# sMedX/FaceNet

Hardware: AMD Instinct MI355X
Metric: images/sec (160x160 triplet train) (higher is better)
Workload: dtype bf16

## Files before the change

facenet_amd/csrc/common.h:

```cpp
#pragma once
#include <hip/hip_runtime.h>
#include <stdint.h>
#include <atomic>
#include <cstdlib>

namespace fn {

enum { FN_OK = 0, FN_EINVAL = -1, FN_ELAUNCH = -2, FN_EUNSUPPORTED = -3 };
void set_error(const char* fmt, ...);
int check_launch(const char* what);

#define FN_REQUIRE(cond, ...)                  \
    do {                                       \
        if (!(cond)) {                         \
            fn::set_error(__VA_ARGS__);        \
            return fn::FN_EINVAL;              \
        }                                      \
    } while (0)

typedef __attribute__((ext_vector_type(8))) __bf16 bf16x8;
typedef __attribute__((ext_vector_type(4))) __bf16 bf16x4;
typedef __attribute__((ext_vector_type(8))) _Float16 f16x8;
typedef __attribute__((ext_vector_type(4))) _Float16 f16x4;
typedef __attribute__((ext_vector_type(4))) float f32x4;
// ... 31 lines not shown
    static __device__ __forceinline__ f32x4 mfma(vec8 a, vec8 b, f32x4 c) {
        return __builtin_amdgcn_mfma_f32_16x16x32_f16(a, b, c, 0, 0, 0);
    }
};

template <typename T> __device__ __forceinline__ void unpack8(const u32x4& v, float (&f)[8]) {
#pragma unroll
    for (int i = 0; i < 4; ++i) {
        f[2 * i] = LP<T>::to_f32((unsigned short)(v[i] & 0xffffu));
        f[2 * i + 1] = LP<T>::to_f32((unsigned short)(v[i] >> 16));
    }
}
template <typename T> __device__ __forceinline__ u32x4 pack8(const float (&f)[8]) {
    u32x4 v;
#pragma unroll
    for (int i = 0; i < 4; ++i)
        v[i] = (unsigned)LP<T>::from_f32(f[2 * i]) | ((unsigned)LP<T>::from_f32(f[2 * i + 1]) << 16);
    return v;
}

__device__ __forceinline__ void fast_divmod(int m, int d, float inv, int& q, int& r) {
    q = (int)((float)m * inv);
    r = m - q * d;
    const int lo = r < 0 ? 1 : 0, hi = r >= d ? 1 : 0;
    q += hi - lo;
    r += (lo - hi) * d;
}

__device__ __forceinline__ float wave_sum(float v) {
#pragma unroll
    for (int o = 32; o > 0; o >>= 1) v += __shfl_xor(v, o);
    return v;
}
__device__ __forceinline__ float wave_max(float v) {
#pragma unroll
    for (int o = 32; o > 0; o >>= 1) v = fmaxf(v, __shfl_xor(v, o));
    return v;
}

typedef int64_t acc_t;
enum { ACC_STAT = 20, ACC_GRAD = 40 };
template <int FRAC> __device__ __forceinline__ void acc_add(acc_t* p, float v) {
    atomicAdd(reinterpret_cast<unsigned long long*>(p), (unsigned long long)__double2ll_rn((double)v * (double)(1ll << FRAC)));
}
template <int FRAC> __device__ __forceinline__ float acc_get(acc_t a) { return (float)((double)a * (1.0 / (double)(1ll << FRAC))); }

__device__ __forceinline__ void bn_affine_from_sums(float s1, float s2, int count, float eps, float beta, float& scale, float& shift,
                                                    float& mean, float& var) {
#pragma clang fp contract(off)
    const float inv = 1.f / (float)count;
    mean = s1 * inv;
    const float ex2 = s2 * inv, m2 = mean * mean;
    var = fmaxf(ex2 - m2, 0.f);
    scale = rsqrtf(var + eps);
    const float ms = mean * scale;
    shift = beta - ms;
}

__device__ __forceinline__ float bn_moving_update(float moving, float batch, float momentum) {
#pragma clang fp contract(off)
    const float a = moving * momentum, w = 1.f - momentum;
    const float b = batch * w;
    return a + b;
}

__device__ __forceinline__ void bn_batch_affine(const acc_t* __restrict__ stats, int c, int sq_off, int reps, int rep_stride, int count,
                                                float eps, float beta, float& scale, float& shift, float& mean, float& var) {
    acc_t s = 0, q = 0;
    for (int rp = 0; rp < reps; ++rp) {
        s += stats[(long)rp * rep_stride + c];
        q += stats[(long)rp * rep_stride + sq_off + c];
    }
    bn_affine_from_sums(acc_get<ACC_STAT>(s), acc_get<ACC_STAT>(q), count, eps, beta, scale, shift, mean, var);
}

enum { STORE_WT = 17 };
// ... 48 lines not shown
```

facenet_amd/csrc/elementwise.hip:

```cpp
#include "common.h"
#include "../../include/facenet_hip.h"

namespace fn {

__device__ __forceinline__ unsigned f2ord(float f) {
    unsigned u = __float_as_uint(f);
    return (u & 0x80000000u) ? ~u : (u | 0x80000000u);
}
__device__ __forceinline__ float ord2f(unsigned u) {
    return __uint_as_float((u & 0x80000000u) ? (u & 0x7fffffffu) : ~u);
}

template <typename SRC>
__global__ __launch_bounds__(256) void img_stats_kernel(const SRC* __restrict__ img, unsigned* __restrict__ work, int count) {
    const int n = blockIdx.y;
    const SRC* p = img + (long)n * count;
    float mx = -3e38f, mn = 3e38f, s = 0.f, q = 0.f;
    constexpr int PER = 16 / sizeof(SRC);
    const int head = min(count, (int)(((16 - ((uintptr_t)p & 15)) & 15) / sizeof(SRC)));
    const int nvec = (count - head) / PER;
    const SRC* pv = p + head;
    for (int i = blockIdx.x * 256 + threadIdx.x; i < nvec; i += gridDim.x * 256) {
        const u32x4 v = *reinterpret_cast<const u32x4*>(pv + (long)i * PER);
#pragma unroll
        for (int w = 0; w < 4; ++w) {
            if constexpr (sizeof(SRC) == 1) {
#pragma unroll
                for (int b = 0; b < 4; ++b) {
                    const float x = (float)((v[w] >> (8 * b)) & 0xffu);
                    mx = fmaxf(mx, x); mn = fminf(mn, x); s += x; q += x * x;
                }
            } else {
                const float x = __uint_as_float(v[w]);
                mx = fmaxf(mx, x); mn = fminf(mn, x); s += x; q += x * x;
            }
        }
    }
    if (blockIdx.x == 0) {
        for (int i = threadIdx.x; i < head; i += 256) {
            const float x = (float)p[i];
            mx = fmaxf(mx, x); mn = fminf(mn, x); s += x; q += x * x;
        }
        for (int i = head + nvec * PER + threadIdx.x; i < count; i += 256) {
            const float x = (float)p[i];
            mx = fmaxf(mx, x); mn = fminf(mn, x); s += x; q += x * x;
        }
    }
    mx = wave_max(mx); mn = -wave_max(-mn); s = wave_sum(s); q = wave_sum(q);
    if ((threadIdx.x & 63) == 0) {
        atomicMax(&work[8 * n + 0], f2ord(mx));
        atomicMax(&work[8 * n + 1], f2ord(-mn));
        acc_add<ACC_STAT>(reinterpret_cast<acc_t*>(&work[8 * n + 2]), s);
        acc_add<ACC_STAT>(reinterpret_cast<acc_t*>(&work[8 * n + 4]), q);
    }
}

template <typename T, typename SRC>
__global__ __launch_bounds__(256) void img_apply_kernel(const SRC* __restrict__ img, unsigned short* __restrict__ out,
                                                        const unsigned* __restrict__ work, int HW, int mode) {
    const int n = blockIdx.y;
    float mul, sub, den;
    if (mode == 0) {
        const float mx = ord2f(work[8 * n + 0]), mn = -ord2f(work[8 * n + 1]);
        mul = 2.f; sub = mn + mx; den = fmaxf(mx - mn, 1e-3f);
    } else {
        const float cnt = (float)HW * 3.f;
        const float mean = acc_get<ACC_STAT>(*reinterpret_cast<const acc_t*>(&work[8 * n + 2])) / cnt;
        const float var = fmaxf(acc_get<ACC_STAT>(*reinterpret_cast<const acc_t*>(&work[8 * n + 4])) / cnt - mean * mean, 0.f);
        mul = 1.f; sub = mean; den = fmaxf(sqrtf(var), rsqrtf(cnt));
    }
    const SRC* p = img + (long)n * HW * 3;
    unsigned short* o = out + (long)n * HW * 8;
    for (int px = blockIdx.x * 256 + threadIdx.x; px < HW; px += gridDim.x * 256) {
        float v[8] = {0, 0, 0, 0, 0, 0, 0, 0};
#pragma unroll
        for (int c = 0; c < 3; ++c) v[c] = (mul * (float)p[px * 3 + c] - sub) / den;
        *reinterpret_cast<u32x4*>(o + (long)px * 8) = pack8<T>(v);
    }
}

template <typename SRC>
__global__ __launch_bounds__(256) void resize_bilinear_kernel(const SRC* __restrict__ img, float* __restrict__ out, int N, int H, int W,
                                                              int OH, int OW) {
    const float sy = (float)H / (float)OH, sx = (float)W / (float)OW;
    const long total = (long)N * OH * OW;
    for (long t = (long)blockIdx.x * 256 + threadIdx.x; t < total; t += (long)gridDim.x * 256) {
        const int ox = (int)(t % OW);
        const int oy = (int)((t / OW) % OH);
        const int n = (int)(t / ((long)OW * OH));
        const float fy = ((float)oy + 0.5f) * sy - 0.5f, fx = ((float)ox + 0.5f) * sx - 0.5f;
        const float fy0 = floorf(fy), fx0 = floorf(fx);
        const int y0 = max((int)fy0, 0), y1 = min((int)ceilf(fy), H - 1);
        const int x0 = max((int)fx0, 0), x1 = min((int)ceilf(fx), W - 1);
        const float ly = fy - fy0, lx = fx - fx0;
        const SRC* p = img + (long)n * H * W * 3;
#pragma unroll
        for (int c = 0; c < 3; ++c) {
            const float v00 = (float)p[((long)y0 * W + x0) * 3 + c], v01 = (float)p[((long)y0 * W + x1) * 3 + c];
            const float v10 = (float)p[((long)y1 * W + x0) * 3 + c], v11 = (float)p[((long)y1 * W + x1) * 3 + c];
            const float top = v00 + (v01 - v00) * lx, bot = v10 + (v11 - v10) * lx;
            out[t * 3 + c] = top + (bot - top) * ly;
        }
    }
}

__global__ __launch_bounds__(256) void gather_images_kernel(const uint8_t* __restrict__ pool, const int32_t* __restrict__ idx,
                                                            uint8_t* __restrict__ out, int bytes) {
    const int i = blockIdx.y;
    const uint8_t* s = pool + (long)idx[i] * bytes;
    uint8_t* d = out + (long)i * bytes;
// ... 618 lines not shown
    }
}

template <typename T> __global__ __launch_bounds__(256) void cast_kernel(const float* __restrict__ x, unsigned short* __restrict__ y, long n) {
    for (long i = (long)blockIdx.x * 256 + threadIdx.x; i < n; i += (long)gridDim.x * 256) y[i] = LP<T>::from_f32(x[i]);
}

static inline int reduce_rows_per_block(int M, int C) {
    int chunks = 32768 / (C > 0 ? C : 1);
    if (chunks < 8) chunks = 8;
    if (chunks > 1024) chunks = 1024;
    int rpb = cdiv(M, chunks);
    if (rpb < 32) rpb = 32;
    return rpb;
}

static inline int grid_for(long work_items, int per_block = 256, int cap = 4096) {
    long g = (work_items + per_block - 1) / per_block;
    if (g < 1) g = 1;
    if (g > cap) g = cap;
    return (int)g;
}

}

using namespace fn;
#define DT_CHECK(dt) FN_REQUIRE((dt) == FN_BF16 || (dt) == FN_F16, "dtype %d unsupported", (dt))
#define LAUNCH_T(dt, KERN, grid, block, smem, st, ...)                                             \
    do {                                                                                             \
        if ((dt) == FN_BF16) hipLaunchKernelGGL(KERN<__bf16>, grid, block, smem, st, __VA_ARGS__);   \
        else hipLaunchKernelGGL(KERN<_Float16>, grid, block, smem, st, __VA_ARGS__);                 \
    } while (0)

template <typename SRC>
static int image_normalize_impl(const SRC* img, void* out, float* work, int N, int HW, int mode, int dtype, void* stream) {
    DT_CHECK(dtype);
    FN_REQUIRE(img && out && work && N > 0 && HW > 0, "image_normalize: bad arguments");
    FN_REQUIRE(mode == 0 || mode == 1, "Invalid image normalization algorithm");
    FN_REQUIRE(((uintptr_t)img % sizeof(SRC)) == 0, "image_normalize: misaligned images");
    hipStream_t st = (hipStream_t)stream;
    fill_words(work, 0u, 0u, 8 * N, st);
    hipLaunchKernelGGL(img_stats_kernel<SRC>, dim3(8, N), dim3(256), 0, st, img, (unsigned*)work, HW * 3);
    const int gx = grid_for(HW, 256, 32);
    if (dtype == FN_BF16) hipLaunchKernelGGL((img_apply_kernel<__bf16, SRC>), dim3(gx, N), dim3(256), 0, st, img, (unsigned short*)out, (const unsigned*)work, HW, mode);
    else hipLaunchKernelGGL((img_apply_kernel<_Float16, SRC>), dim3(gx, N), dim3(256), 0, st, img, (unsigned short*)out, (const unsigned*)work, HW, mode);
    return check_launch("image_normalize");
}
extern "C" int fn_image_normalize(const uint8_t* img, void* out, float* work, int N, int HW, int mode, int dtype, void* stream) {
    return image_normalize_impl<uint8_t>(img, out, work, N, HW, mode, dtype, stream);
}
extern "C" int fn_image_normalize_f32(const float* img, void* out, float* work, int N, int HW, int mode, int dtype, void* stream) {
    return image_normalize_impl<float>(img, out, work, N, HW, mode, dtype, stream);
}

extern "C" int fn_image_resize_bilinear(const void* img, int src_is_f32, float* out, int N, int H, int W, int OH, int OW, void* stream) {
    FN_REQUIRE(img && out && N > 0 && H > 0 && W > 0 && OH > 0 && OW > 0, "image_resize: bad arguments");
    const int grid = grid_for((long)N * OH * OW);
    if (src_is_f32) hipLaunchKernelGGL(resize_bilinear_kernel<float>, dim3(grid), dim3(256), 0, (hipStream_t)stream, (const float*)img, out, N, H, W, OH, OW);
    else hipLaunchKernelGGL(resize_bilinear_kernel<uint8_t>, dim3(grid), dim3(256), 0, (hipStream_t)stream, (const uint8_t*)img, out, N, H, W, OH, OW);
    return check_launch("image_resize");
}

__global__ __launch_bounds__(256) void crop_or_pad_kernel(const uint8_t* __restrict__ src, const long long* __restrict__ off,
                                                          const int* __restrict__ hw, uint8_t* __restrict__ dst, int S) {
    const int n = blockIdx.y;
    const int h = hw[2 * n], w = hw[2 * n + 1];
    const int cy = max((h - S) / 2, 0), cx = max((w - S) / 2, 0);
    const int py = max((S - h) / 2, 0), px = max((S - w) / 2, 0);
    const int ch = min(h, S), cw = min(w, S);
    const uint8_t* im = src + off[n];
    const int words = S * S * 3 / 4;
    for (int t = blockIdx.x * 256 + threadIdx.x; t < words; t += gridDim.x * 256) {
        unsigned v = 0;
#pragma unroll
        for (int b = 0; b < 4; ++b) {
// ... 213 lines not shown
```

facenet_amd/csrc/loss.hip:

```cpp
#include "pair_tiles.h"
#include "../../include/facenet_hip.h"

namespace fn {

__global__ __launch_bounds__(256) void pairwise_kernel(const float* __restrict__ xa, const float* __restrict__ xb, float* __restrict__ out,
                                                       int* __restrict__ range, int n, int m, int E, int metric) {
    const int lane = threadIdx.x & 63, wave = threadIdx.x >> 6;
    const int i = blockIdx.y;
    const int jb = (blockIdx.x * 4 + wave) * 16;
    if (jb >= m) return;
    float a[8];
#pragma unroll
    for (int t = 0; t < 8; ++t) a[t] = (lane + 64 * t < E) ? xa[(long)i * E + lane + 64 * t] : 0.f;
    float asq = 0.f;
#pragma unroll
    for (int t = 0; t < 8; ++t) asq = __fmaf_rn(a[t], a[t], asq);
    asq = wave_sum(asq);
    DotRange seen;
    for (int j = jb; j < min(m, jb + 16); ++j) {
        float d = 0.f, bsq = 0.f;
#pragma unroll
        for (int t = 0; t < 8; ++t) {
            const float b = (lane + 64 * t < E) ? xb[(long)j * E + lane + 64 * t] : 0.f;
            d = __fmaf_rn(a[t], b, d);
            bsq = __fmaf_rn(b, b, bsq);
        }
        d = wave_sum(d);
        float r;
        if (metric == 2) {
            bsq = wave_sum(bsq);
            r = fmaxf(__fmaf_rn(-2.f, d, asq + bsq), 0.f);
        } else {
            seen.add(d);
            r = pair_distance(d, metric);
        }
        if (lane == 0) out[(long)i * m + j] = r;
    }
    if (range && lane == 0 && metric != 2) seen.write(range);
}

__device__ __forceinline__ unsigned hash_mix(unsigned h, unsigned v) {
    h ^= v;
    h ^= h >> 16;
    h *= 0x7FEB352Du;
    h ^= h >> 15;
    h *= 0x846CA68Bu;
    h ^= h >> 16;
    return h;
}
__device__ __forceinline__ unsigned hash_u32(unsigned a, unsigned b, unsigned c) {
    return hash_mix(hash_mix(hash_mix(0x9E3779B9u, a), b), c);
}

__global__ __launch_bounds__(1024) void select_pairs_kernel(const int* __restrict__ labels, int n, int* __restrict__ info) {
    __shared__ int s_lab[1024];
    __shared__ int s_off[1025];
    const int tid = threadIdx.x;
    int* rec = info + 8;
    for (int i = tid; i < n; i += 1024) s_lab[i] = labels[i];
    __syncthreads();
    int cnt = 0;
    if (tid < n)
        for (int p = tid + 1; p < n; ++p) cnt += (s_lab[p] == s_lab[tid]);
    {
        __shared__ int s_wtot[16];
        const int lane = tid & 63, wv = tid >> 6;
        int v = tid < n ? cnt : 0;
#pragma unroll
        for (int d = 1; d < 64; d <<= 1) {
            const int u = __shfl_up(v, d);
            if (lane >= d) v += u;
        }
        if (lane == 63) s_wtot[wv] = v;
        __syncthreads();
        int carry = 0;
        for (int w = 0; w < wv; ++w) carry += s_wtot[w];
        if (tid < n) s_off[tid + 1] = v + carry;
        if (tid == 0) s_off[0] = 0;
    }
    __syncthreads();
    if (tid < n) {
        int q = s_off[tid];
        for (int p = tid + 1; p < n; ++p)
            if (s_lab[p] == s_lab[tid]) { rec[5 * q + 0] = tid; rec[5 * q + 1] = p; ++q; }
    }
    if (tid == 0) {
        info[0] = s_off[n];
        info[1] = 0;
    }
}

__global__ __launch_bounds__(256) void select_negatives_kernel(const float* __restrict__ dist, const int* __restrict__ labels, int n,
                                                               float alpha, unsigned seed0, int semi_hard, int* __restrict__ info) {
    const int lane = threadIdx.x & 63;
    const int q = blockIdx.x * 4 + (threadIdx.x >> 6);
    if (q >= info[0]) return;
    const unsigned seed = seed0 + (unsigned)info[3];
    int* rec = info + 8;
    const int a = rec[5 * q + 0], p = rec[5 * q + 1];
    const int la = labels[a];
    const float dap = dist[(long)p * n + a];
    int c = 0, others = 0;
    for (int j0 = 0; j0 < n; j0 += 64) {
        const int j = j0 + lane;
        const bool oth = (j < n) && (labels[j] != la);
        const float daj = oth ? dist[(long)j * n + a] : 0.f;
        const bool cand = oth && (daj - dap < alpha) && (!semi_hard || daj > dap);
        c += __popcll(__ballot(cand));
        others += __popcll(__ballot(oth));
    }
    const bool use_cand = c > 0;
    int want = use_cand ? (int)(hash_u32(seed, (unsigned)q, 0u) % (unsigned)c)
                        : (others > 0 ? (int)(hash_u32(seed, (unsigned)q, 2u) % (unsigned)others) : -1);
    int neg = -1;
    for (int j0 = 0; j0 < n && want >= 0; j0 += 64) {
        const int j = j0 + lane;
        const bool oth = (j < n) && (labels[j] != la);
        const float daj = oth ? dist[(long)j * n + a] : 0.f;
        const bool hit = use_cand ? (oth && (daj - dap < alpha) && (!semi_hard || daj > dap)) : oth;
        const unsigned long long m = __ballot(hit);
        const int cnt = __popcll(m);
        if (want < cnt) {
            const int rank = __popcll(m & ((1ull << lane) - 1ull));
            const unsigned long long sel = __ballot(hit && rank == want);
            neg = j0 + (int)__ffsll((long long)sel) - 1;
            want = -1;
        } else {
            want -= cnt;
        }
    }
    if (lane == 0) {
        rec[5 * q + 2] = neg;
        rec[5 * q + 3] = (int)hash_u32(seed, (unsigned)q, 1u);
        rec[5 * q + 4] = use_cand ? 0 : 1;
        if (use_cand) atomicAdd(&info[1], 1);
    }
}

__global__ __launch_bounds__(1024) void select_rank_kernel(int T, int* __restrict__ triplets, int* __restrict__ info) {
    const int tid = threadIdx.x;
    const int* rec = info + 8;
    const int Q = info[0];
    __shared__ unsigned long long s_key[4096];
    for (int q = tid; q < min(Q, 4096); q += 1024)
        s_key[q] = ((unsigned long long)(unsigned)rec[5 * q + 4] << 32) | (unsigned)rec[5 * q + 3];
    __syncthreads();
    for (int q = tid; q < Q; q += 1024) {
        const int cls = rec[5 * q + 4];
        const unsigned key = (unsigned)rec[5 * q + 3];
        const unsigned long long mine = ((unsigned long long)(unsigned)cls << 32) | key;
        int rank = 0;
        const int QL = min(Q, 4096);
        for (int r = 0; r < QL; ++r) {
            const unsigned long long k2 = s_key[r];
            rank += (k2 < mine || (k2 == mine && r < q)) ? 1 : 0;
        }
        for (int r = QL; r < Q; ++r) {
            const int c2 = rec[5 * r + 4];
            const unsigned k2 = (unsigned)rec[5 * r + 3];
            const bool before = (c2 < cls) || (c2 == cls && (k2 < key || (k2 == key && r < q)));
            rank += before ? 1 : 0;
        }
        if (rank < T && rec[5 * q + 2] >= 0) {
            triplets[3 * rank + 0] = rec[5 * q + 0];
            triplets[3 * rank + 1] = rec[5 * q + 1];
            triplets[3 * rank + 2] = rec[5 * q + 2];
        }
    }
    if (tid == 0) {
        info[2] = (Q < T) ? 1 : 0;
        info[3] = info[3] + 1;
    }
}

__global__ __launch_bounds__(256) void triplet_loss_kernel(const float* __restrict__ emb, float* __restrict__ demb, acc_t* __restrict__ loss,
                                                           int T, int E, float alpha) {
    const int t = blockIdx.x * 4 + (threadIdx.x >> 6), lane = threadIdx.x & 63;
    if (t >= T) return;
    const float* a = emb + (long)(3 * t) * E;
    const float* p = a + E;
    const float* ng = p + E;
    float pos = 0.f, neg = 0.f;
    for (int k = lane; k < E; k += 64) {
        const float dp = a[k] - p[k], dn = a[k] - ng[k];
        pos += dp * dp;
        neg += dn * dn;
    }
    pos = wave_sum(pos);
    neg = wave_sum(neg);
    const float l = pos - neg + alpha;
    const float on = l > 0.f ? 1.f : 0.f;
    if (lane == 0) acc_add<ACC_GRAD>(loss, fmaxf(l, 0.f) / (float)T);
    if (demb) {
        const float s = 2.f * on / (float)T;
        float* da = demb + (long)(3 * t) * E;
        for (int k = lane; k < E; k += 64) {
            da[k] = s * (ng[k] - p[k]);
            da[E + k] = s * (p[k] - a[k]);
            da[2 * E + k] = s * (a[k] - ng[k]);
        }
    }
}

template <typename T>
__global__ __launch_bounds__(256) void softmax_xent_kernel(const float* __restrict__ logits, int ld, const int* __restrict__ labels,
                                                           acc_t* __restrict__ loss, unsigned short* __restrict__ dlogits, int ld_d,
                                                           acc_t* __restrict__ dbias, int N, int C, float grad_scale) {
    __shared__ float red[4];
    const int row = blockIdx.x, tid = threadIdx.x, lane = tid & 63, wave = tid >> 6;
    const float* x = logits + (long)row * ld;
    float mx = -3e38f;
    for (int c = tid; c < C; c += 256) mx = fmaxf(mx, x[c]);
    mx = wave_max(mx);
    if (lane == 0) red[wave] = mx;
    __syncthreads();
    mx = fmaxf(fmaxf(red[0], red[1]), fmaxf(red[2], red[3]));
    __syncthreads();
    float s = 0.f;
    for (int c = tid; c < C; c += 256) s += __expf(x[c] - mx);
    s = wave_sum(s);
    if (lane == 0) red[wave] = s;
    __syncthreads();
    s = red[0] + red[1] + red[2] + red[3];
    const int lab = labels[row];
    const bool lab_ok = lab >= 0 && lab < C;
    if (tid == 0) {
        if (lab_ok) acc_add<ACC_GRAD>(loss, (logf(s) + mx - x[lab]) / (float)N);
        else reinterpret_cast<volatile unsigned*>(loss)[-1] = 1u;
    }
    if (dlogits) {
        const float inv = 1.f / s;
        unsigned short* d = dlogits + (long)row * ld_d;
        for (int c = tid; c < ld_d; c += 256) {
// ... 254 lines not shown
    const float* wr = w + (long)j * E;
    float* dr = dw + (long)j * E;
    for (int e = 4 * lane; e < E; e += 256) {
        const f32x4 wv = *reinterpret_cast<const f32x4*>(wr + e);
        f32x4 dv = *reinterpret_cast<const f32x4*>(dr + e);
#pragma unroll
        for (int t = 0; t < 4; ++t) {
            const float p = kf * wv[t];
            dv[t] = dv[t] - p;
        }
        *reinterpret_cast<f32x4*>(dr + e) = dv;
    }
}
}
using namespace fn;

extern "C" int fn_pairwise_sqdist(const float* xa, const float* xb, float* out, float* range, int n, int m, int E, int metric, void* stream) {
    FN_REQUIRE(xa && xb && out && n > 0 && m > 0 && E > 0 && E <= 512, "pairwise_sqdist: bad arguments (E must be <= 512)");
    FN_REQUIRE(metric >= 0 && metric <= 2, "Undefined similarity metric %d", metric);
    hipStream_t st = (hipStream_t)stream;
    if (range) {
        fill_words(range, 0x7f7fffffu, 0x80800000u, 2, st);
    }
    hipLaunchKernelGGL(pairwise_kernel, dim3(cdiv(m, 64), n), dim3(256), 0, st, xa, xb, out, (int*)range, n, m, E, metric);
    return check_launch("pairwise_sqdist");
}

extern "C" int fn_select_triplets(const float* dist, const int32_t* labels, int n, float alpha, int nrof_triplets, uint32_t seed,
                                  int semi_hard, int32_t* triplets, int32_t* info, void* stream) {
    FN_REQUIRE(dist && labels && triplets && info && n > 1 && n <= 1024 && nrof_triplets > 0, "select_triplets: bad arguments (n <= 1024)");
    hipStream_t st = (hipStream_t)stream;
    hipLaunchKernelGGL(select_pairs_kernel, dim3(1), dim3(1024), 0, st, labels, n, info);
    const int max_pairs = n * (n - 1) / 2;
    hipLaunchKernelGGL(select_negatives_kernel, dim3(cdiv(max_pairs, 4)), dim3(256), 0, st, dist, labels, n, alpha, seed, semi_hard, info);
    hipLaunchKernelGGL(select_rank_kernel, dim3(1), dim3(1024), 0, st, nrof_triplets, triplets, info);
    return check_launch("select_triplets");
}

extern "C" int fn_triplet_loss_fwd_bwd(const float* emb, float* demb, float* loss, int T, int E, float alpha, void* stream) {
    FN_REQUIRE(emb && loss && T > 0 && E > 0, "triplet_loss: bad arguments");
    hipStream_t st = (hipStream_t)stream;
    FN_REQUIRE(((uintptr_t)loss & 7) == 0, "triplet_loss: loss must be an 8-byte aligned fp32[4]");
    fill_words(loss, 0u, 0u, 4, st);
    hipLaunchKernelGGL(triplet_loss_kernel, dim3(cdiv(T, 4)), dim3(256), 0, st, emb, demb, reinterpret_cast<acc_t*>(loss + 2), T, E, alpha);
    hipLaunchKernelGGL(loss_finish_kernel, dim3(1), dim3(1), 0, st, loss);
    return check_launch("triplet_loss");
}

extern "C" int fn_softmax_xent_fwd_bwd(const float* logits, int ld, const int32_t* labels, float* loss, void* dlogits_lp, int ld_d, fn_acc_t* dbias_,
                                       int N, int C, float grad_scale, int dtype, void* stream) {
    acc_t* dbias = reinterpret_cast<acc_t*>(dbias_);
    FN_REQUIRE(((uintptr_t)loss & 7) == 0, "softmax_xent: loss must be an 8-byte aligned fp32[4]");
    FN_REQUIRE(dtype == FN_BF16 || dtype == FN_F16, "dtype %d unsupported", dtype);
    FN_REQUIRE(logits && labels && loss && N > 0 && C > 0 && ld >= C && (!dlogits_lp || ld_d >= C), "softmax_xent: bad arguments");
    hipStream_t st = (hipStream_t)stream;
    fill_words(loss, 0u, 0u, 4, st);
    acc_t* lacc = reinterpret_cast<acc_t*>(loss + 2);
    if (dtype == FN_BF16)
        hipLaunchKernelGGL(softmax_xent_kernel<__bf16>, dim3(N), dim3(256), 0, st, logits, ld, labels, lacc, (unsigned short*)dlogits_lp, ld_d, dbias, N, C, grad_scale);
    else
        hipLaunchKernelGGL(softmax_xent_kernel<_Float16>, dim3(N), dim3(256), 0, st, logits, ld, labels, lacc, (unsigned short*)dlogits_lp, ld_d, dbias, N, C, grad_scale);
    hipLaunchKernelGGL(loss_finish_kernel, dim3(1), dim3(1), 0, st, loss);
    return check_launch("softmax_xent");
}

extern "C" int fn_center_loss_fwd_bwd(const float* x, const int32_t* labels, const float* centers, float* demb, float* terms, float* xy,
                                      int ld_xy, int N, int E, int C, float center_factor, float norm_factor, float p, void* stream) {
    FN_REQUIRE(x && labels && terms && N > 0 && E > 0 && E % 4 == 0, "center_loss: bad arguments (E must be a multiple of 4)");
    FN_REQUIRE(((uintptr_t)x & 15) == 0 && (!demb || ((uintptr_t)demb & 15) == 0) && (!centers || ((uintptr_t)centers & 15) == 0),
               "center_loss: x, demb and centers must be 16-byte aligned");
    FN_REQUIRE(((uintptr_t)terms & 7) == 0, "center_loss: terms must be an 8-byte aligned fp32[8]");
    FN_REQUIRE(!centers || C > 0, "center_loss: centers need C > 0");
    FN_REQUIRE(!xy || ld_xy > E, "center_loss: ld_xy must be > E");
    FN_REQUIRE(center_factor >= 0.f && norm_factor >= 0.f && p > 0.f, "center_loss: factors must be >= 0 and p > 0");
    hipStream_t st = (hipStream_t)stream;
// ... 50 lines not shown
```

Measured before the change: 14110.

## Fuse image normalize, triplet selection and loss kernels to cut launches

Image normalization now runs as one kernel per image that stages the image in LDS, computes statistics and applies the affine transform, with a lookup table for 8-bit inputs. This replaces the separate fill, stats and apply launches. Negative selection and ranking are merged into one kernel that uses a last-block ticket, and pair counting uses wave ballots. The pairwise distance loop batches four wave reductions. Small triplet counts use a single-block loss kernel without the fill and finish launches. These cut launch overhead and serialization in the non-GEMM pipeline stages, but they add complexity and lower parallelism per image (one block).

```diff
diff --git a/facenet_amd/csrc/common.h b/facenet_amd/csrc/common.h
--- a/facenet_amd/csrc/common.h
+++ b/facenet_amd/csrc/common.h
@@ -87,6 +87,16 @@
     for (int o = 32; o > 0; o >>= 1) v += __shfl_xor(v, o);
     return v;
 }
+template <int N> __device__ __forceinline__ void wave_sum_n(float (&v)[N]) {
+#pragma unroll
+    for (int o = 32; o > 0; o >>= 1) {
+        float u[N];
+#pragma unroll
+        for (int k = 0; k < N; ++k) u[k] = __shfl_xor(v[k], o);
+#pragma unroll
+        for (int k = 0; k < N; ++k) v[k] += u[k];
+    }
+}
 __device__ __forceinline__ float wave_max(float v) {
 #pragma unroll
     for (int o = 32; o > 0; o >>= 1) v = fmaxf(v, __shfl_xor(v, o));
@@ -95,8 +105,9 @@
 
 typedef int64_t acc_t;
 enum { ACC_STAT = 20, ACC_GRAD = 40 };
+template <int FRAC> __device__ __forceinline__ acc_t acc_fixed(float v) { return __double2ll_rn((double)v * (double)(1ll << FRAC)); }
 template <int FRAC> __device__ __forceinline__ void acc_add(acc_t* p, float v) {
-    atomicAdd(reinterpret_cast<unsigned long long*>(p), (unsigned long long)__double2ll_rn((double)v * (double)(1ll << FRAC)));
+    atomicAdd(reinterpret_cast<unsigned long long*>(p), (unsigned long long)acc_fixed<FRAC>(v));
 }
 template <int FRAC> __device__ __forceinline__ float acc_get(acc_t a) { return (float)((double)a * (1.0 / (double)(1ll << FRAC))); }
 
diff --git a/facenet_amd/csrc/elementwise.hip b/facenet_amd/csrc/elementwise.hip
--- a/facenet_amd/csrc/elementwise.hip
+++ b/facenet_amd/csrc/elementwise.hip
@@ -10,72 +10,165 @@
 __device__ __forceinline__ float ord2f(unsigned u) {
     return __uint_as_float((u & 0x80000000u) ? (u & 0x7fffffffu) : ~u);
 }
+
+struct ImgStat {
+    float mx = -3e38f, mn = 3e38f, s = 0.f, q = 0.f;
+    __device__ __forceinline__ void add(float x) { mx = fmaxf(mx, x); mn = fminf(mn, x); s += x; q += x * x; }
+    template <typename SRC> __device__ __forceinline__ void add_vec(const u32x4& v) {
+#pragma unroll
+        for (int w = 0; w < 4; ++w) {
+            if constexpr (sizeof(SRC) == 1) {
+#pragma unroll
+                for (int b = 0; b < 4; ++b) add((float)((v[w] >> (8 * b)) & 0xffu));
+            } else {
+                add(__uint_as_float(v[w]));
+            }
+        }
+    }
+    __device__ __forceinline__ void reduce_wave() { mx = wave_max(mx); mn = -wave_max(-mn); s = wave_sum(s); q = wave_sum(q); }
+};
+
+template <typename SRC> __device__ __forceinline__ int img_head(const SRC* p, int count) {
+    return min(count, (int)(((16 - ((uintptr_t)p & 15)) & 15) / sizeof(SRC)));
+}
+
+enum { IMG_STAT_THREADS = 2048, IMG_STAT_WAVES = IMG_STAT_THREADS / 64, IMG_STAT_LDS = IMG_STAT_WAVES * 24,
+       IMG_TABLE_LDS = 256 * 2 };
 
 template <typename SRC>
 __global__ __launch_bounds__(256) void img_stats_kernel(const SRC* __restrict__ img, unsigned* __restrict__ work, int count) {
     const int n = blockIdx.y;
     const SRC* p = img + (long)n * count;
-    float mx = -3e38f, mn = 3e38f, s = 0.f, q = 0.f;
+    ImgStat st;
     constexpr int PER = 16 / sizeof(SRC);
-    const int head = min(count, (int)(((16 - ((uintptr_t)p & 15)) & 15) / sizeof(SRC)));
+    const int head = img_head(p, count);
     const int nvec = (count - head) / PER;
     const SRC* pv = p + head;
-    for (int i = blockIdx.x * 256 + threadIdx.x; i < nvec; i += gridDim.x * 256) {
-        const u32x4 v = *reinterpret_cast<const u32x4*>(pv + (long)i * PER);
-#pragma unroll
-        for (int w = 0; w < 4; ++w) {
-            if constexpr (sizeof(SRC) == 1) {
-#pragma unroll
-                for (int b = 0; b < 4; ++b) {
-                    const float x = (float)((v[w] >> (8 * b)) & 0xffu);
-                    mx = fmaxf(mx, x); mn = fminf(mn, x); s += x; q += x * x;
-                }
-            } else {
-                const float x = __uint_as_float(v[w]);
-                mx = fmaxf(mx, x); mn = fminf(mn, x); s += x; q += x * x;
-            }
-        }
-    }
+    for (int i = blockIdx.x * 256 + threadIdx.x; i < nvec; i += gridDim.x * 256)
+        st.template add_vec<SRC>(*reinterpret_cast<const u32x4*>(pv + (long)i * PER));
     if (blockIdx.x == 0) {
-        for (int i = threadIdx.x; i < head; i += 256) {
-            const float x = (float)p[i];
-            mx = fmaxf(mx, x); mn = fminf(mn, x); s += x; q += x * x;
-        }
-        for (int i = head + nvec * PER + threadIdx.x; i < count; i += 256) {
-            const float x = (float)p[i];
-            mx = fmaxf(mx, x); mn = fminf(mn, x); s += x; q += x * x;
-        }
-    }
-    mx = wave_max(mx); mn = -wave_max(-mn); s = wave_sum(s); q = wave_sum(q);
+        for (int i = threadIdx.x; i < head; i += 256) st.add((float)p[i]);
+        for (int i = head + nvec * PER + threadIdx.x; i < count; i += 256) st.add((float)p[i]);
+    }
+    st.reduce_wave();
     if ((threadIdx.x & 63) == 0) {
-        atomicMax(&work[8 * n + 0], f2ord(mx));
-        atomicMax(&work[8 * n + 1], f2ord(-mn));
-        acc_add<ACC_STAT>(reinterpret_cast<acc_t*>(&work[8 * n + 2]), s);
-        acc_add<ACC_STAT>(reinterpret_cast<acc_t*>(&work[8 * n + 4]), q);
-    }
-}
+        atomicMax(&work[8 * n + 0], f2ord(st.mx));
+        atomicMax(&work[8 * n + 1], f2ord(-st.mn));
+        acc_add<ACC_STAT>(reinterpret_cast<acc_t*>(&work[8 * n + 2]), st.s);
+        acc_add<ACC_STAT>(reinterpret_cast<acc_t*>(&work[8 * n + 4]), st.q);
+    }
+}
+
+struct ImgAffine {
+    float mul, sub, den;
+    __device__ __forceinline__ ImgAffine(unsigned omx, unsigned omn, acc_t s, acc_t q, int HW, int mode) {
+        if (mode == 0) {
+            const float mx = ord2f(omx), mn = -ord2f(omn);
+            mul = 2.f; sub = mn + mx; den = fmaxf(mx - mn, 1e-3f);
+        } else {
+            const float cnt = (float)HW * 3.f;
+            const float mean = acc_get<ACC_STAT>(s) / cnt;
+            const float var = fmaxf(acc_get<ACC_STAT>(q) / cnt - mean * mean, 0.f);
+            mul = 1.f; sub = mean; den = fmaxf(sqrtf(var), rsqrtf(cnt));
+        }
+    }
+    template <typename T, typename SRC> __device__ __forceinline__ u32x4 pixel(const SRC* p) const {
+        float v[8] = {0, 0, 0, 0, 0, 0, 0, 0};
+#pragma unroll
+        for (int c = 0; c < 3; ++c) v[c] = value((float)p[c]);
+        return pack8<T>(v);
+    }
+    __device__ __forceinline__ float value(float x) const { return (mul * x - sub) / den; }
+};
 
 template <typename T, typename SRC>
 __global__ __launch_bounds__(256) void img_apply_kernel(const SRC* __restrict__ img, unsigned short* __restrict__ out,
                                                         const unsigned* __restrict__ work, int HW, int mode) {
     const int n = blockIdx.y;
-    float mul, sub, den;
-    if (mode == 0) {
-        const float mx = ord2f(work[8 * n + 0]), mn = -ord2f(work[8 * n + 1]);
-        mul = 2.f; sub = mn + mx; den = fmaxf(mx - mn, 1e-3f);
-    } else {
-        const float cnt = (float)HW * 3.f;
-        const float mean = acc_get<ACC_STAT>(*reinterpret_cast<const acc_t*>(&work[8 * n + 2])) / cnt;
-        const float var = fmaxf(acc_get<ACC_STAT>(*reinterpret_cast<const acc_t*>(&work[8 * n + 4])) / cnt - mean * mean, 0.f);
-        mul = 1.f; sub = mean; den = fmaxf(sqrtf(var), rsqrtf(cnt));
-    }
+    const ImgAffine af(work[8 * n + 0], work[8 * n + 1], *reinterpret_cast<const acc_t*>(&work[8 * n + 2]),
+                       *reinterpret_cast<const acc_t*>(&work[8 * n + 4]), HW, mode);
     const SRC* p = img + (long)n * HW * 3;
     unsigned short* o = out + (long)n * HW * 8;
-    for (int px = blockIdx.x * 256 + threadIdx.x; px < HW; px += gridDim.x * 256) {
-        float v[8] = {0, 0, 0, 0, 0, 0, 0, 0};
-#pragma unroll
-        for (int c = 0; c < 3; ++c) v[c] = (mul * (float)p[px * 3 + c] - sub) / den;
-        *reinterpret_cast<u32x4*>(o + (long)px * 8) = pack8<T>(v);
+    for (int px = blockIdx.x * 256 + threadIdx.x; px < HW; px += gridDim.x * 256)
+        *reinterpret_cast<u32x4*>(o + (long)px * 8) = af.template pixel<T, SRC>(p + px * 3);
+}
+
+template <typename T, typename SRC>
+__global__ __launch_bounds__(1024) void img_normalize_kernel(const SRC* __restrict__ img, unsigned short* __restrict__ out,
+                                                             unsigned* __restrict__ work, int HW, int mode) {
+    extern __shared__ u32x4 s_lds[];
+    acc_t* s_s = reinterpret_cast<acc_t*>(s_lds);
+    acc_t* s_q = s_s + IMG_STAT_WAVES;
+    unsigned* s_mx = reinterpret_cast<unsigned*>(s_q + IMG_STAT_WAVES);
+    unsigned* s_mn = s_mx + IMG_STAT_WAVES;
+    unsigned short* s_tab = reinterpret_cast<unsigned short*>(s_lds + IMG_STAT_LDS / 16);
+    u32x4* s_img4 = s_lds + (IMG_STAT_LDS + IMG_TABLE_LDS) / 16;
+    const int n = blockIdx.x, tid = threadIdx.x, lane = tid & 63;
+    const int count = HW * 3;
+    const SRC* p = img + (long)n * count;
+    constexpr int PER = 16 / sizeof(SRC);
+    const int head = img_head(p, count);
+    const int nvec = (count - head) / PER;
+    SRC* s_el = reinterpret_cast<SRC*>(s_img4) + ((uintptr_t)p & 15) / sizeof(SRC);
+    u32x4* s_vec = reinterpret_cast<u32x4*>(s_el + head);
+    const u32x4* pv = reinterpret_cast<const u32x4*>(p + head);
+    for (int i0 = tid; i0 < nvec; i0 += 5 * 1024) {
+        u32x4 r[5];
+#pragma unroll
+        for (int k = 0; k < 5; ++k) r[k] = (i0 + 1024 * k < nvec) ? pv[i0 + 1024 * k] : u32x4{0u, 0u, 0u, 0u};
+#pragma unroll
+        for (int k = 0; k < 5; ++k)
+            if (i0 + 1024 * k < nvec) s_vec[i0 + 1024 * k] = r[k];
+    }
+    if (tid < 256) {
+        for (int i = tid; i < head; i += 256) s_el[i] = p[i];
+        for (int i = head + nvec * PER + tid; i < count; i += 256) s_el[i] = p[i];
+    }
+#pragma unroll
+    for (int half = 0; half < 2; ++half) {
+        const int vt = tid + 1024 * half;
+        ImgStat st;
+        for (int i = vt; i < nvec; i += IMG_STAT_THREADS) st.template add_vec<SRC>(s_vec[i]);
+        if (vt < 256) {
+            for (int i = vt; i < head; i += 256) st.add((float)s_el[i]);
+            for (int i = head + nvec * PER + vt; i < count; i += 256) st.add((float)s_el[i]);
+        }
+        st.reduce_wave();
+        if (lane == 0) {
+            const int w = vt >> 6;
+            s_mx[w] = f2ord(st.mx);
+            s_mn[w] = f2ord(-st.mn);
+            s_s[w] = acc_fixed<ACC_STAT>(st.s);
+            s_q[w] = acc_fixed<ACC_STAT>(st.q);
+        }
+    }
+    __syncthreads();
+    unsigned omx = 0u, omn = 0u;
+    acc_t ss = 0, qq = 0;
+#pragma unroll
+    for (int w = 0; w < IMG_STAT_WAVES; ++w) {
+        omx = max(omx, s_mx[w]); omn = max(omn, s_mn[w]);
+        ss += s_s[w]; qq += s_q[w];
+    }
+    if (tid == 0) {
+        unsigned* w = work + 8 * n;
+        w[0] = omx; w[1] = omn;
+        *reinterpret_cast<acc_t*>(w + 2) = ss;
+        *reinterpret_cast<acc_t*>(w + 4) = qq;
+        w[6] = 0u; w[7] = 0u;
+    }
+    const ImgAffine af(omx, omn, ss, qq, HW, mode);
+    unsigned short* o = out + (long)n * HW * 8;
+    if constexpr (sizeof(SRC) == 1) {
+        if (tid < 256) s_tab[tid] = LP<T>::from_f32(af.value((float)tid));
+        __syncthreads();
+        for (int px = tid; px < HW; px += 1024) {
+            const SRC* e = s_el + px * 3;
+            *reinterpret_cast<u32x4*>(o + (long)px * 8) = u32x4{(unsigned)s_tab[e[0]] | ((unsigned)s_tab[e[1]] << 16), (unsigned)s_tab[e[2]], 0u, 0u};
+        }
+    } else {
+        for (int px = tid; px < HW; px += 1024)
+            *reinterpret_cast<u32x4*>(o + (long)px * 8) = af.template pixel<T, SRC>(s_el + px * 3);
     }
 }
 
@@ -760,6 +853,8 @@
         else hipLaunchKernelGGL(KERN<_Float16>, grid, block, smem, st, __VA_ARGS__);                 \
     } while (0)
 
+enum { IMG_LDS_MAX_BYTES = 158 * 1024 };
+
 template <typename SRC>
 static int image_normalize_impl(const SRC* img, void* out, float* work, int N, int HW, int mode, int dtype, void* stream) {
     DT_CHECK(dtype);
@@ -767,8 +862,19 @@
     FN_REQUIRE(mode == 0 || mode == 1, "Invalid image normalization algorithm");
     FN_REQUIRE(((uintptr_t)img % sizeof(SRC)) == 0, "image_normalize: misaligned images");
     hipStream_t st = (hipStream_t)stream;
+    const long bytes = (long)HW * 3 * sizeof(SRC);
+    if (bytes <= IMG_LDS_MAX_BYTES) {
+        const size_t smem = IMG_STAT_LDS + IMG_TABLE_LDS + 16 + (size_t)((bytes + 15) & ~15l);
+        static LdsOptIn lds_ok[2];
+        const bool bf = dtype == FN_BF16;
+        const void* kern = bf ? reinterpret_cast<const void*>(img_normalize_kernel<__bf16, SRC>) : reinterpret_cast<const void*>(img_normalize_kernel<_Float16, SRC>);
+        if (int rc = allow_big_lds(kern, lds_ok[bf ? 0 : 1], "image_normalize")) return rc;
+        if (bf) hipLaunchKernelGGL((img_normalize_kernel<__bf16, SRC>), dim3(N), dim3(1024), smem, st, img, (unsigned short*)out, (unsigned*)work, HW, mode);
+        else hipLaunchKernelGGL((img_normalize_kernel<_Float16, SRC>), dim3(N), dim3(1024), smem, st, img, (unsigned short*)out, (unsigned*)work, HW, mode);
+        return check_launch("image_normalize");
+    }
     fill_words(work, 0u, 0u, 8 * N, st);
-    hipLaunchKernelGGL(img_stats_kernel<SRC>, dim3(8, N), dim3(256), 0, st, img, (unsigned*)work, HW * 3);
+    hipLaunchKernelGGL(img_stats_kernel<SRC>, dim3(IMG_STAT_THREADS / 256, N), dim3(256), 0, st, img, (unsigned*)work, HW * 3);
     const int gx = grid_for(HW, 256, 32);
     if (dtype == FN_BF16) hipLaunchKernelGGL((img_apply_kernel<__bf16, SRC>), dim3(gx, N), dim3(256), 0, st, img, (unsigned short*)out, (const unsigned*)work, HW, mode);
     else hipLaunchKernelGGL((img_apply_kernel<_Float16, SRC>), dim3(gx, N), dim3(256), 0, st, img, (unsigned short*)out, (const unsigned*)work, HW, mode);
diff --git a/facenet_amd/csrc/loss.hip b/facenet_amd/csrc/loss.hip
--- a/facenet_amd/csrc/loss.hip
+++ b/facenet_amd/csrc/loss.hip
@@ -17,24 +17,35 @@
     for (int t = 0; t < 8; ++t) asq = __fmaf_rn(a[t], a[t], asq);
     asq = wave_sum(asq);
     DotRange seen;
-    for (int j = jb; j < min(m, jb + 16); ++j) {
-        float d = 0.f, bsq = 0.f;
-#pragma unroll
-        for (int t = 0; t < 8; ++t) {
-            const float b = (lane + 64 * t < E) ? xb[(long)j * E + lane + 64 * t] : 0.f;
-            d = __fmaf_rn(a[t], b, d);
-            bsq = __fmaf_rn(b, b, bsq);
-        }
-        d = wave_sum(d);
-        float r;
-        if (metric == 2) {
-            bsq = wave_sum(bsq);
-            r = fmaxf(__fmaf_rn(-2.f, d, asq + bsq), 0.f);
-        } else {
-            seen.add(d);
-            r = pair_distance(d, metric);
-        }
-        if (lane == 0) out[(long)i * m + j] = r;
+    constexpr int JU = 4;
+    const int jend = min(m, jb + 16);
+    for (int j0 = jb; j0 < jend; j0 += JU) {
+        float d[JU], bsq[JU];
+#pragma unroll
+        for (int u = 0; u < JU; ++u) {
+            const int j = min(j0 + u, jend - 1);
+            d[u] = 0.f; bsq[u] = 0.f;
+#pragma unroll
+            for (int t = 0; t < 8; ++t) {
+                const float b = (lane + 64 * t < E) ? xb[(long)j * E + lane + 64 * t] : 0.f;
+                d[u] = __fmaf_rn(a[t], b, d[u]);
+                bsq[u] = __fmaf_rn(b, b, bsq[u]);
+            }
+        }
+        wave_sum_n(d);
+        if (metric == 2) wave_sum_n(bsq);
+#pragma unroll
+        for (int u = 0; u < JU; ++u) {
+            if (j0 + u >= jend) break;
+            float r;
+            if (metric == 2) {
+                r = fmaxf(__fmaf_rn(-2.f, d[u], asq + bsq[u]), 0.f);
+            } else {
+                seen.add(d[u]);
+                r = pair_distance(d[u], metric);
+            }
+            if (lane == 0) out[(long)i * m + j0 + u] = r;
+        }
     }
     if (range && lane == 0 && metric != 2) seen.write(range);
 }
@@ -52,20 +63,29 @@
     return hash_mix(hash_mix(hash_mix(0x9E3779B9u, a), b), c);
 }
 
+enum { SEL_TICKET = 4, SEL_WAVES = 16, SEL_MAX_GROUPS = 64 };
+
 __global__ __launch_bounds__(1024) void select_pairs_kernel(const int* __restrict__ labels, int n, int* __restrict__ info) {
     __shared__ int s_lab[1024];
+    __shared__ int s_cnt[1024];
     __shared__ int s_off[1025];
-    const int tid = threadIdx.x;
+    const int tid = threadIdx.x, lane = tid & 63, wv = tid >> 6;
     int* rec = info + 8;
     for (int i = tid; i < n; i += 1024) s_lab[i] = labels[i];
     __syncthreads();
-    int cnt = 0;
-    if (tid < n)
-        for (int p = tid + 1; p < n; ++p) cnt += (s_lab[p] == s_lab[tid]);
+    for (int a = wv; a < n; a += SEL_WAVES) {
+        const int la = s_lab[a];
+        int cnt = 0;
+        for (int p0 = (a + 1) & ~63; p0 < n; p0 += 64) {
+            const int p = p0 + lane;
+            cnt += __popcll(__ballot(p > a && p < n && s_lab[p] == la));
+        }
+        if (lane == 0) s_cnt[a] = cnt;
+    }
+    __syncthreads();
     {
         __shared__ int s_wtot[16];
-        const int lane = tid & 63, wv = tid >> 6;
-        int v = tid < n ? cnt : 0;
+        int v = tid < n ? s_cnt[tid] : 0;
 #pragma unroll
         for (int d = 1; d < 64; d <<= 1) {
             const int u = __shfl_up(v, d);
@@ -79,10 +99,20 @@
         if (tid == 0) s_off[0] = 0;
     }
     __syncthreads();
-    if (tid < n) {
-        int q = s_off[tid];
-        for (int p = tid + 1; p < n; ++p)
-            if (s_lab[p] == s_lab[tid]) { rec[5 * q + 0] = tid; rec[5 * q + 1] = p; ++q; }
+    for (int a = wv; a < n; a += SEL_WAVES) {
+        const int la = s_lab[a];
+        int q = s_off[a];
+        for (int p0 = (a + 1) & ~63; p0 < n; p0 += 64) {
+            const int p = p0 + lane;
+            const bool hit = p > a && p < n && s_lab[p] == la;
+            const unsigned long long m = __ballot(hit);
+            if (hit) {
+                const int qq = q + __popcll(m & ((1ull << lane) - 1ull));
+                rec[5 * qq + 0] = a;
+                rec[5 * qq + 1] = p;
+            }
+            q += __popcll(m);
+        }
     }
     if (tid == 0) {
         info[0] = s_off[n];
@@ -90,42 +120,59 @@
     }
 }
 
-__global__ __launch_bounds__(256) void select_negatives_kernel(const float* __restrict__ dist, const int* __restrict__ labels, int n,
-                                                               float alpha, unsigned seed0, int semi_hard, int* __restrict__ info) {
-    const int lane = threadIdx.x & 63;
-    const int q = blockIdx.x * 4 + (threadIdx.x >> 6);
-    if (q >= info[0]) return;
-    const unsigned seed = seed0 + (unsigned)info[3];
+template <int NG>
+__device__ __forceinline__ void select_negative(const float* __restrict__ dist, const int* __restrict__ labels, int n, float alpha,
+                                                unsigned seed, int semi_hard, int q, int lane, int* __restrict__ info) {
     int* rec = info + 8;
     const int a = rec[5 * q + 0], p = rec[5 * q + 1];
     const int la = labels[a];
     const float dap = dist[(long)p * n + a];
+    unsigned long long m_oth[4 * NG], m_cand[4 * NG];
+#pragma unroll
+    for (int g = 0; g < NG; ++g) {
+        if (g * 256 < n) {
+            int lab[4];
+            float daj[4];
+#pragma unroll
+            for (int k = 0; k < 4; ++k) {
+                const int j = min((g * 4 + k) * 64 + lane, n - 1);
+                lab[k] = labels[j];
+                daj[k] = dist[(long)j * n + a];
+            }
+#pragma unroll
+            for (int k = 0; k < 4; ++k) {
+                const bool oth = ((g * 4 + k) * 64 + lane < n) && (lab[k] != la);
+                const bool cand = oth && (daj[k] - dap < alpha) && (!semi_hard || daj[k] > dap);
+                m_oth[g * 4 + k] = __ballot(oth);
+                m_cand[g * 4 + k] = __ballot(cand);
+            }
+        } else {
+#pragma unroll
+            for (int k = 0; k < 4; ++k) m_oth[g * 4 + k] = m_cand[g * 4 + k] = 0ull;
+        }
+    }
     int c = 0, others = 0;
-    for (int j0 = 0; j0 < n; j0 += 64) {
-        const int j = j0 + lane;
-        const bool oth = (j < n) && (labels[j] != la);
-        const float daj = oth ? dist[(long)j * n + a] : 0.f;
-        const bool cand = oth && (daj - dap < alpha) && (!semi_hard || daj > dap);
-        c += __popcll(__ballot(cand));
-        others += __popcll(__ballot(oth));
+#pragma unroll
+    for (int b = 0; b < 4 * NG; ++b) {
+        c += __popcll(m_cand[b]);
+        others += __popcll(m_oth[b]);
     }
     const bool use_cand = c > 0;
     int want = use_cand ? (int)(hash_u32(seed, (unsigned)q, 0u) % (unsigned)c)
                         : (others > 0 ? (int)(hash_u32(seed, (unsigned)q, 2u) % (unsigned)others) : -1);
     int neg = -1;
-    for (int j0 = 0; j0 < n && want >= 0; j0 += 64) {
-        const int j = j0 + lane;
-        const bool oth = (j < n) && (labels[j] != la);
-        const float daj = oth ? dist[(long)j * n + a] : 0.f;
-        const bool hit = use_cand ? (oth && (daj - dap < alpha) && (!semi_hard || daj > dap)) : oth;
-        const unsigned long long m = __ballot(hit);
+    const unsigned long long all_others = use_cand ? 0ull : ~0ull;
+#pragma unroll
+    for (int b = 0; b < 4 * NG; ++b) {
+        const unsigned long long m = m_oth[b] & (m_cand[b] | all_others);
         const int cnt = __popcll(m);
-        if (want < cnt) {
+        if (want >= 0 && want < cnt) {
+            const bool hit = (m >> lane) & 1ull;
             const int rank = __popcll(m & ((1ull << lane) - 1ull));
             const unsigned long long sel = __ballot(hit && rank == want);
-            neg = j0 + (int)__ffsll((long long)sel) - 1;
+            neg = b * 64 + (int)__ffsll((long long)sel) - 1;
             want = -1;
-        } else {
+        } else if (want >= 0) {
             want -= cnt;
         }
     }
@@ -137,20 +184,17 @@
     }
 }
 
-__global__ __launch_bounds__(1024) void select_rank_kernel(int T, int* __restrict__ triplets, int* __restrict__ info) {
-    const int tid = threadIdx.x;
-    const int* rec = info + 8;
-    const int Q = info[0];
-    __shared__ unsigned long long s_key[4096];
-    for (int q = tid; q < min(Q, 4096); q += 1024)
+__device__ __forceinline__ void select_rank(int T, int Q, int* __restrict__ triplets, const int* rec, unsigned long long* s_key) {
+    const int tid = threadIdx.x, nth = blockDim.x;
+    const int QL = min(Q, 4096);
+    for (int q = tid; q < QL; q += nth)
         s_key[q] = ((unsigned long long)(unsigned)rec[5 * q + 4] << 32) | (unsigned)rec[5 * q + 3];
     __syncthreads();
-    for (int q = tid; q < Q; q += 1024) {
+    for (int q = tid; q < Q; q += nth) {
         const int cls = rec[5 * q + 4];
         const unsigned key = (unsigned)rec[5 * q + 3];
         const unsigned long long mine = ((unsigned long long)(unsigned)cls << 32) | key;
         int rank = 0;
-        const int QL = min(Q, 4096);
         for (int r = 0; r < QL; ++r) {
             const unsigned long long k2 = s_key[r];
             rank += (k2 < mine || (k2 == mine && r < q)) ? 1 : 0;
@@ -167,16 +211,43 @@
             triplets[3 * rank + 2] = rec[5 * q + 2];
         }
     }
+}
+
+template <int NG>
+__global__ __launch_bounds__(1024) void select_negatives_rank_kernel(const float* __restrict__ dist, const int* __restrict__ labels, int n,
+                                                                     float alpha, unsigned seed0, int semi_hard, int T,
+                                                                     int* __restrict__ triplets, int* __restrict__ info) {
+    __shared__ unsigned long long s_key[4096];
+    __shared__ int s_last;
+    const int tid = threadIdx.x, lane = tid & 63;
+    const int Q = info[0];
+    const unsigned seed = seed0 + (unsigned)info[3];
+    for (int q = blockIdx.x * SEL_WAVES + (tid >> 6); q < Q; q += gridDim.x * SEL_WAVES)
+        select_negative<NG>(dist, labels, n, alpha, seed, semi_hard, q, lane, info);
+    asm volatile("s_waitcnt vmcnt(0)" ::: "memory");
+    __syncthreads();
+    if (tid == 0) {
+        __builtin_amdgcn_fence(__ATOMIC_RELEASE, "agent");
+        asm volatile("s_waitcnt vmcnt(0)" ::: "memory");
+        const int ticket = __hip_atomic_fetch_add(&info[SEL_TICKET], 1, __ATOMIC_RELAXED, __HIP_MEMORY_SCOPE_AGENT);
+        const int last = ticket == (int)gridDim.x - 1;
+        if (last) {
+            __builtin_amdgcn_fence(__ATOMIC_ACQUIRE, "agent");
+            asm volatile("s_waitcnt vmcnt(0)" ::: "memory");
+        }
+        s_last = last;
+    }
+    __syncthreads();
+    if (!s_last) return;
+    select_rank(T, Q, triplets, info + 8, s_key);
     if (tid == 0) {
         info[2] = (Q < T) ? 1 : 0;
         info[3] = info[3] + 1;
-    }
-}
-
-__global__ __launch_bounds__(256) void triplet_loss_kernel(const float* __restrict__ emb, float* __restrict__ demb, acc_t* __restrict__ loss,
-                                                           int T, int E, float alpha) {
-    const int t = blockIdx.x * 4 + (threadIdx.x >> 6), lane = threadIdx.x & 63;
-    if (t >= T) return;
+        info[SEL_TICKET] = 0;
+    }
+}
+
+__device__ __forceinline__ float triplet_term(const float* __restrict__ emb, float* __restrict__ demb, int t, int lane, int T, int E, float alpha) {
     const float* a = emb + (long)(3 * t) * E;
     const float* p = a + E;
     const float* ng = p + E;
@@ -190,7 +261,6 @@
     neg = wave_sum(neg);
     const float l = pos - neg + alpha;
     const float on = l > 0.f ? 1.f : 0.f;
-    if (lane == 0) acc_add<ACC_GRAD>(loss, fmaxf(l, 0.f) / (float)T);
     if (demb) {
         const float s = 2.f * on / (float)T;
         float* da = demb + (long)(3 * t) * E;
@@ -199,6 +269,35 @@
             da[E + k] = s * (p[k] - a[k]);
             da[2 * E + k] = s * (a[k] - ng[k]);
         }
+    }
+    return fmaxf(l, 0.f) / (float)T;
+}
+
+__global__ __launch_bounds__(256) void triplet_loss_kernel(const float* __restrict__ emb, float* __restrict__ demb, acc_t* __restrict__ loss,
+                                                           int T, int E, float alpha) {
+    const int t = blockIdx.x * 4 + (threadIdx.x >> 6), lane = threadIdx.x & 63;
+    if (t >= T) return;
+    const float term = triplet_term(emb, demb, t, lane, T, E, alpha);
+    if (lane == 0) acc_add<ACC_GRAD>(loss, term);
+}
+
+enum { TRIPLET_ONE_GROUP = 64 };
+__global__ __launch_bounds__(1024) void triplet_loss_one_group_kernel(const float* __restrict__ emb, float* __restrict__ demb,
+                                                                      float* __restrict__ loss, int T, int E, float alpha) {
+    __shared__ unsigned long long s_acc;
+    const int tid = threadIdx.x, lane = tid & 63;
+    if (tid == 0) s_acc = 0ull;
+    __syncthreads();
+    for (int t = tid >> 6; t < T; t += 16) {
+        const float term = triplet_term(emb, demb, t, lane, T, E, alpha);
+        if (lane == 0) atomicAdd(&s_acc, (unsigned long long)acc_fixed<ACC_GRAD>(term));
+    }
+    __syncthreads();
+    if (tid == 0) {
+        const acc_t sum = (acc_t)s_acc;
+        loss[0] = acc_get<ACC_GRAD>(sum);
+        reinterpret_cast<unsigned*>(loss)[1] = 0u;
+        *reinterpret_cast<acc_t*>(loss + 2) = sum;
     }
 }
 
@@ -519,8 +618,10 @@
     hipStream_t st = (hipStream_t)stream;
     hipLaunchKernelGGL(select_pairs_kernel, dim3(1), dim3(1024), 0, st, labels, n, info);
     const int max_pairs = n * (n - 1) / 2;
-    hipLaunchKernelGGL(select_negatives_kernel, dim3(cdiv(max_pairs, 4)), dim3(256), 0, st, dist, labels, n, alpha, seed, semi_hard, info);
-    hipLaunchKernelGGL(select_rank_kernel, dim3(1), dim3(1024), 0, st, nrof_triplets, triplets, info);
+    const int groups = min(cdiv(max_pairs, SEL_WAVES), (int)SEL_MAX_GROUPS);
+    auto kern = n <= 256 ? select_negatives_rank_kernel<1> : n <= 512 ? select_negatives_rank_kernel<2> : n <= 768 ? select_negatives_rank_kernel<3>
+                                                                                                                    : select_negatives_rank_kernel<4>;
+    hipLaunchKernelGGL(kern, dim3(groups), dim3(1024), 0, st, dist, labels, n, alpha, seed, semi_hard, nrof_triplets, triplets, info);
     return check_launch("select_triplets");
 }
 
@@ -528,6 +629,10 @@
     FN_REQUIRE(emb && loss && T > 0 && E > 0, "triplet_loss: bad arguments");
     hipStream_t st = (hipStream_t)stream;
     FN_REQUIRE(((uintptr_t)loss & 7) == 0, "triplet_loss: loss must be an 8-byte aligned fp32[4]");
+    if (T <= TRIPLET_ONE_GROUP) {
+        hipLaunchKernelGGL(triplet_loss_one_group_kernel, dim3(1), dim3(1024), 0, st, emb, demb, loss, T, E, alpha);
+        return check_launch("triplet_loss");
+    }
     fill_words(loss, 0u, 0u, 4, st);
     hipLaunchKernelGGL(triplet_loss_kernel, dim3(cdiv(T, 4)), dim3(256), 0, st, emb, demb, reinterpret_cast<acc_t*>(loss + 2), T, E, alpha);
     hipLaunchKernelGGL(loss_finish_kernel, dim3(1), dim3(1), 0, st, loss);
```

New measurement: 14170, median of 6. Within noise of the previous version (+0.4%).
